# JackShDr/InfluentialRS

Measured on NVIDIA B200. Metric: IRN influence-path generation throughput @1M items, higher is better.
Workload: dtype f32

## Files before the change

influentialrs_b200/csrc/decoder_chain_tc.cu:

```cuda
#include "tc_common.cuh"
#include "qkv_image.cuh"

namespace irs {
namespace tcl {

using namespace irs::tc;

constexpr int BM = 128, D = 128, F = 256;
constexpr int RING = 4;
constexpr uint32_t UNIT_BYTES = 16384, UNIT_HALF = 8192;
constexpr uint32_t A_LBO = BM * 16;
constexpr uint32_t SBO = 128;
constexpr uint32_t OFF_P = 0;
constexpr uint32_t OFF_Q = 65536;
constexpr uint32_t OFF_RING = 131072;
constexpr uint32_t OFF_VEC = OFF_RING + RING * UNIT_BYTES;
constexpr int V_BO = 0, V_G1 = 128, V_B1 = 256, V_C2 = 384, V_G2 = 512, V_B2 = 640, V_BF1 = 768, V_BF2 = 1024,
              V_G3 = 1152, V_B3 = 1280, V_BIN = 1408, V_TOTAL = 1792;
constexpr uint32_t OFF_XCH = OFF_VEC + V_TOTAL * 4;
constexpr uint32_t OFF_BARS = OFF_XCH + 3 * 2 * 128 * 8;
enum Bars { B_FULL = 0, B_EMPTY = 4, B_A0 = 8, B_D1 = 9, B_A1 = 10, B_D2 = 11, B_A2 = 12 , B_D3 = 16,
            B_A3 = 17, B_D4 = 18, B_COUNT = 20 };
constexpr uint32_t OFF_TMEM = OFF_BARS + B_COUNT * 8;
constexpr uint32_t SMEM_BYTES = OFF_TMEM + 16;
constexpr int EPI_WARPS = 8, EPI_THREADS = EPI_WARPS * 32;
constexpr int LOAD_WARPS = 2;
constexpr int WARP_LOAD0 = 8, WARP_PROD = 10, WARP_MMA = 11;
constexpr int THREADS = 12 * 32;
constexpr int UNITS_BODY = 20;
constexpr int UNITS_QKV = 12;
constexpr uint32_t T_H = 0, T_Y = 256, T_D3 = 384;

struct Params {
  const float* attn;
  const float* x;
  float* x_out;
  float* qkv_out;
  uint8_t* qkv_images;
  int L, mask_mode;
  int qkv_only;
  const uint4* wstream;
  const float* vec[11];
  float eps1, eps2, eps3;
  int64_t R; int64_t n_tiles; int n_units;
  int* error_flag;
  long long* timeline;
};

struct UnitDesc { int mat, n0, k0, kind; };
__host__ __device__ inline UnitDesc unit_desc(int u) {
  UnitDesc d;
  if (u < 4) { d.mat = 0; d.n0 = 0; d.k0 = 32 * u; d.kind = 0; }
  else if (u < 12) { d.mat = 1; d.n0 = 0; d.k0 = 16 * (u - 4); d.kind = 2; }
  else if (u < 20) { d.mat = 2; d.n0 = 0; d.k0 = 32 * (u - 12); d.kind = 0; }
  else if (u < 28) { d.mat = 3; d.n0 = 0; d.k0 = 16 * (u - 20); d.kind = 2; }
  else { d.mat = 3; d.n0 = 256; d.k0 = 32 * (u - 28); d.kind = 0; }
  return d;
}

__global__ void __launch_bounds__(256)
prepare_chain_kernel(const float* __restrict__ Wo, const float* __restrict__ W1, const float* __restrict__ W2,
                     const float* __restrict__ Win, int n_units, uint4* __restrict__ out) {
  const int total = n_units * 1024;
  for (int idx = blockIdx.x * blockDim.x + threadIdx.x; idx < total; idx += gridDim.x * blockDim.x) {
    const int u = idx >> 10, w = idx & 1023;
    const int part = w >> 9, rem = w & 511;
    const UnitDesc ud = unit_desc(u);
    int slab, row;
    if (ud.kind == 0) { slab = rem >> 7; row = rem & 127; } else { slab = rem >> 8; row = rem & 255; }
    const float* W; int ldw;
    switch (ud.mat) { case 0: W = Wo; ldw = D; break; case 1: W = W1; ldw = D; break; case 2: W = W2; ldw = F; break;
                      default: W = Win; ldw = D; break; }
    const float* src = W + (int64_t)(ud.n0 + row) * ldw + ud.k0 + slab * 8;
    float x[8];
#pragma unroll
    for (int e = 0; e < 8; ++e) x[e] = src[e];
    uint4 hi, lo;
    split8(x, hi, lo);
    out[idx] = part ? lo : hi;
  }
}

__device__ __forceinline__ void ldg256_nc(const float* p, float (&a)[8]) {
  asm volatile("ld.global.nc.L1::no_allocate.v8.f32 {%0,%1,%2,%3,%4,%5,%6,%7}, [%8];"
               : "=f"(a[0]), "=f"(a[1]), "=f"(a[2]), "=f"(a[3]), "=f"(a[4]), "=f"(a[5]), "=f"(a[6]), "=f"(a[7]) : "l"(p));
}
__device__ __forceinline__ void ldg256(const float* p, float (&a)[8]) {
  asm volatile("ld.global.L1::no_allocate.v8.f32 {%0,%1,%2,%3,%4,%5,%6,%7}, [%8];"
               : "=f"(a[0]), "=f"(a[1]), "=f"(a[2]), "=f"(a[3]), "=f"(a[4]), "=f"(a[5]), "=f"(a[6]), "=f"(a[7]) : "l"(p) : "memory");
}
__device__ __forceinline__ void stg256(float* p, const float* a) {
  asm volatile("st.global.L1::no_allocate.v8.f32 [%0], {%1,%2,%3,%4,%5,%6,%7,%8};"
               :: "l"(p), "f"(a[0]), "f"(a[1]), "f"(a[2]), "f"(a[3]), "f"(a[4]), "f"(a[5]), "f"(a[6]), "f"(a[7]) : "memory");
}
__device__ __forceinline__ void stg128(void* p, const uint4& v) {
  asm volatile("st.global.L1::no_allocate.v4.b32 [%0], {%1,%2,%3,%4};" :: "l"(p), "r"(v.x), "r"(v.y), "r"(v.z), "r"(v.w) : "memory");
}
__device__ __forceinline__ void prefetch_l2_bulk(const void* p, uint32_t bytes) {
  asm volatile("cp.async.bulk.prefetch.L2.global [%0], %1;" :: "l"(p), "r"(bytes) : "memory");
}

template <int KSTEPS>
__device__ __forceinline__ void mma_unit(uint32_t d_tmem, uint32_t a_hi, uint32_t a_lo, uint32_t b_stage, uint32_t b_lbo,
                                         uint32_t idesc, bool first) {
#pragma unroll
  for (int kk = 0; kk < KSTEPS; ++kk) {
    const uint64_t ah = make_desc(a_hi + (uint32_t)(2 * kk) * A_LBO, A_LBO, SBO);
    const uint64_t al = make_desc(a_lo + (uint32_t)(2 * kk) * A_LBO, A_LBO, SBO);
    const uint64_t bh = make_desc(b_stage + (uint32_t)(2 * kk) * b_lbo, b_lbo, SBO);
    const uint64_t bl = make_desc(b_stage + UNIT_HALF + (uint32_t)(2 * kk) * b_lbo, b_lbo, SBO);
    tc_mma_bf16(d_tmem, al, bh, idesc, (first && kk == 0) ? 0u : 1u);
    tc_mma_bf16(d_tmem, ah, bl, idesc, 1u);
    tc_mma_bf16(d_tmem, ah, bh, idesc, 1u);
  }
}

#define IRS_TL(role, idx)                                                                         \
  do {                                                                                            \
    if (p.timeline && blockIdx.x == 0 && it < 8 && lane == 0)                                     \
      p.timeline[(it * 3 + (role)) * 32 + (idx)] = clock64();                                     \
  } while (0)

__device__ __forceinline__ void pair_barrier(int quad) {
  asm volatile("bar.sync %0, 64;" :: "r"(1 + quad) : "memory");
}

__device__ __forceinline__ float2 ln_pair_stats(float (&t)[64], float2* mine, const float2* other, int quad, float eps) {
  float s[4] = {0.f, 0.f, 0.f, 0.f}, q[4] = {0.f, 0.f, 0.f, 0.f};
#pragma unroll
  for (int j = 0; j < 64; ++j) s[j & 3] += t[j];
  const float m = ((s[0] + s[1]) + (s[2] + s[3])) * (1.0f / 64.0f);
#pragma unroll
  for (int j = 0; j < 64; ++j) {
    t[j] -= m;
    q[j & 3] = fmaf(t[j], t[j], q[j & 3]);
  }
  const float qs = (q[0] + q[1]) + (q[2] + q[3]);
  *mine = make_float2(m, qs);
  pair_barrier(quad);
  const float2 o = *other;
  const float delta = o.x - m;
  const float mean = 0.5f * (m + o.x);
  const float rstd = rsqrtf(fmaf(32.f * delta, delta, qs + o.y) * (1.0f / (float)D) + eps);
  return make_float2(rstd, (m - mean) * rstd);
}

__global__ void __launch_bounds__(THREADS, 1)
decoder_chain_kernel(const Params p) {
  extern __shared__ __align__(128) uint8_t smem[];
  const uint32_t sbase = smem_u32(smem);
  const int tid = threadIdx.x, warp = tid >> 5, lane = tid & 31;
  auto bar = [&](int i) { return sbase + OFF_BARS + 8u * (uint32_t)i; };
  volatile uint32_t* tmem_holder = reinterpret_cast<volatile uint32_t*>(smem + OFF_TMEM);
  float* vecs = reinterpret_cast<float*>(smem + OFF_VEC);
  const bool with_qkv = (p.qkv_out != nullptr) || (p.qkv_images != nullptr);
  const bool qkv_only = p.qkv_only != 0;

  if (tid == 0) {
    for (int s = 0; s < RING; ++s) { mbar_init(bar(B_FULL + s), 1); mbar_init(bar(B_EMPTY + s), 1); }
    mbar_init(bar(B_A0), LOAD_WARPS);
    mbar_init(bar(B_D1), 1);
    mbar_init(bar(B_A1), EPI_THREADS);
    mbar_init(bar(B_D2), 1);
    for (int i = 0; i < 4; ++i) mbar_init(bar(B_A2 + i), EPI_THREADS);
    mbar_init(bar(B_D3), 1);
    mbar_init(bar(B_A3), EPI_THREADS);
    for (int i = 0; i < 2; ++i) mbar_init(bar(B_D4 + i), 1);
    asm volatile("fence.mbarrier_init.release.cluster;" ::: "memory");
  }
  if (warp == WARP_MMA) {
    asm volatile("tcgen05.alloc.cta_group::1.sync.aligned.shared::cta.b32 [%0], %1;" :: "r"(sbase + OFF_TMEM), "r"(512u) : "memory");
    asm volatile("tcgen05.relinquish_alloc_permit.cta_group::1.sync.aligned;" ::: "memory");
  }
  {
    const int vlen[11] = {128, 128, 128, 128, 128, 128, 256, 128, 128, 128, 384};
    int off = 0;
    const float qscale0 = 1.4426950408889634f / sqrtf((float)img::DH);
    for (int v = 0; v < 11; ++v) {
      for (int i = tid; i < vlen[v]; i += THREADS) {
        float x = p.vec[v] ? p.vec[v][i] : 0.f;
        if (v == 2 && p.vec[3]) x += p.vec[3][i];
        if (v == 10 && p.qkv_images && i < D) x *= qscale0;
        vecs[off + i] = x;
      }
      off += vlen[v];
    }
  }
  tc_fence_before();
  __syncthreads();
  tc_fence_after();
  const uint32_t tmem_base = *tmem_holder;
  const int64_t first_tile = blockIdx.x, tile_step = gridDim.x;

  if (warp >= WARP_LOAD0 && warp < WARP_LOAD0 + LOAD_WARPS) {
    const int lw = warp - WARP_LOAD0;
    const int r8 = lane & 7, sg = lane >> 3;
    const uint32_t a0_off = qkv_only ? OFF_P : OFF_Q;
    int it = 0;
    for (int64_t tile = first_tile; tile < p.n_tiles; tile += tile_step, ++it) {
      const int64_t r0 = tile * BM;
#pragma unroll 1
      for (int batch = 0; batch < 64 / LOAD_WARPS / 8; ++batch) {
        float v[8][8];
#pragma unroll
        for (int q = 0; q < 8; ++q) {
          const int qq = batch * 8 + q;
          const int row = (lw * (16 / LOAD_WARPS) + (qq >> 2)) * 8 + r8;
          const int slab = (qq & 3) * 4 + sg;
          if (r0 + row < p.R) ldg256_nc(p.attn + (r0 + row) * D + slab * 8, v[q]);
          else {
#pragma unroll
            for (int e = 0; e < 8; ++e) v[q][e] = 0.f;
          }
        }
        if (batch == 0 && lw == 0) IRS_TL(2, 0);
        if (batch == 0 && it > 0) mbar_wait(bar(qkv_only ? B_D4 + 1 : B_D3), (uint32_t)((it - 1) & 1), p.error_flag, 31);
        if (batch == 0 && lw == 0) IRS_TL(2, 1);
#pragma unroll
        for (int q = 0; q < 8; ++q) {
          const int qq = batch * 8 + q;
          const int row = (lw * (16 / LOAD_WARPS) + (qq >> 2)) * 8 + r8;
          const int slab = (qq & 3) * 4 + sg;
          uint4 hi, lo;
          split8(v[q], hi, lo);
          *reinterpret_cast<uint4*>(smem + a0_off + slab * A_LBO + row * 16) = hi;
          *reinterpret_cast<uint4*>(smem + a0_off + 32768 + slab * A_LBO + row * 16) = lo;
        }
      }
      asm volatile("fence.proxy.async.shared::cta;" ::: "memory");
      __syncwarp();
      if (lane == 0) mbar_arrive(bar(B_A0));
      if (lw == 0) IRS_TL(2, 2);
    }
  } else if (warp == WARP_PROD) {
    if (lane == 0) {
      int64_t g = 0;
      for (int64_t tile = first_tile; tile < p.n_tiles; tile += tile_step) {
        const int64_t nt = tile + tile_step;
        if (nt < p.n_tiles) {
          const int64_t rows = (p.R - nt * BM) < BM ? (p.R - nt * BM) : BM;
          if (p.x) prefetch_l2_bulk(p.x + nt * BM * D, (uint32_t)(rows * D * 4));
          prefetch_l2_bulk(p.attn + nt * BM * D, (uint32_t)(rows * D * 4));
        }
        for (int u = 0; u < p.n_units; ++u, ++g) {
          const int stage = (int)(g % RING);
          const uint32_t phase = (uint32_t)((g / RING) & 1);
          mbar_wait(bar(B_EMPTY + stage), phase ^ 1u, p.error_flag, 32);
          mbar_arrive_expect_tx(bar(B_FULL + stage), UNIT_BYTES);
          bulk_g2s(sbase + OFF_RING + stage * UNIT_BYTES, p.wstream + (int64_t)u * (UNIT_BYTES / 16), UNIT_BYTES, bar(B_FULL + stage));
        }
      }
    }
  } else if (warp == WARP_MMA) {
    if (lane == 0) {
      const uint32_t idesc128 = make_idesc_bf16(BM, 128), idesc256 = make_idesc_bf16(BM, 256);
      const uint32_t P_HI = sbase + OFF_P, P_LO = sbase + OFF_P + 32768, Q_HI = sbase + OFF_Q, Q_LO = sbase + OFF_Q + 32768;
      int64_t g = 0;
      auto next_unit = [&]() -> uint32_t {
        const int stage = (int)(g % RING);
        mbar_wait(bar(B_FULL + stage), (uint32_t)((g / RING) & 1), p.error_flag, 33);
        tc_fence_after();
        return sbase + OFF_RING + stage * UNIT_BYTES;
      };
      auto release_unit = [&]() { tc_commit(bar(B_EMPTY + (int)(g % RING))); ++g; };
      int it = 0;
      for (int64_t tile = first_tile; tile < p.n_tiles; tile += tile_step, ++it) {
        const uint32_t ph = (uint32_t)(it & 1);
        if (qkv_only) {
          mbar_wait(bar(B_A0), ph, p.error_flag, 34);
          if (it > 0) mbar_wait(bar(B_A1), (uint32_t)((it - 1) & 1), p.error_flag, 38);
          tc_fence_after();
          for (int u = 0; u < 8; ++u) {
            const uint32_t bs = next_unit();
            mma_unit<1>(tmem_base + T_H, P_HI + (uint32_t)(2 * u) * A_LBO, P_LO + (uint32_t)(2 * u) * A_LBO, bs, 4096u, idesc256, u == 0);
            release_unit();
          }
          tc_commit(bar(B_D4 + 0));
          for (int c = 0; c < 4; ++c) {
            const uint32_t bs = next_unit();
            mma_unit<2>(tmem_base + T_D3, P_HI + (uint32_t)(4 * c) * A_LBO, P_LO + (uint32_t)(4 * c) * A_LBO, bs, 2048u, idesc128, c == 0);
            release_unit();
          }
          tc_commit(bar(B_D4 + 1));
          continue;
        }
        IRS_TL(0, 0);
        mbar_wait(bar(B_A0), ph, p.error_flag, 34);
        tc_fence_after();
        IRS_TL(0, 1);
        for (int c = 0; c < 4; ++c) {
          const uint32_t bs = next_unit();
          mma_unit<2>(tmem_base + T_Y, Q_HI + (uint32_t)(4 * c) * A_LBO, Q_LO + (uint32_t)(4 * c) * A_LBO, bs, 2048u, idesc128, c == 0);
          release_unit();
        }
        tc_commit(bar(B_D1));
        IRS_TL(0, 2);
        mbar_wait(bar(B_A1), ph, p.error_flag, 35);
        tc_fence_after();
        IRS_TL(0, 3);
        for (int u = 0; u < 8; ++u) {
          const uint32_t bs = next_unit();
          mma_unit<1>(tmem_base + T_H, P_HI + (uint32_t)(2 * u) * A_LBO, P_LO + (uint32_t)(2 * u) * A_LBO, bs, 4096u, idesc256, u == 0);
          release_unit();
        }
        tc_commit(bar(B_D2));
        for (int j = 0; j < 4; ++j) {
          IRS_TL(0, 4 + 2 * j);
          mbar_wait(bar(B_A2 + j), ph, p.error_flag, 36);
          tc_fence_after();
          IRS_TL(0, 5 + 2 * j);
          const uint32_t slot = (j < 2 ? Q_HI : P_HI) + (uint32_t)(j & 1) * 32768u;
          for (int i = 0; i < 2; ++i) {
            const uint32_t bs = next_unit();
            mma_unit<2>(tmem_base + T_D3, slot + (uint32_t)(4 * i) * A_LBO, slot + 16384u + (uint32_t)(4 * i) * A_LBO, bs,
                        2048u, idesc128, j == 0 && i == 0);
            release_unit();
          }
        }
        tc_commit(bar(B_D3));
        IRS_TL(0, 12);
        mbar_wait(bar(B_A3), ph, p.error_flag, 37);
        tc_fence_after();
        IRS_TL(0, 13);
        if (with_qkv) {
          for (int u = 0; u < 8; ++u) {
            const uint32_t bs = next_unit();
            mma_unit<1>(tmem_base + T_H, P_HI + (uint32_t)(2 * u) * A_LBO, P_LO + (uint32_t)(2 * u) * A_LBO, bs, 4096u, idesc256, u == 0);
            release_unit();
          }
          tc_commit(bar(B_D4 + 0));
          IRS_TL(0, 14);
          for (int c = 0; c < 4; ++c) {
            const uint32_t bs = next_unit();
            mma_unit<2>(tmem_base + T_D3, P_HI + (uint32_t)(4 * c) * A_LBO, P_LO + (uint32_t)(4 * c) * A_LBO, bs, 2048u, idesc128, c == 0);
            release_unit();
          }
          tc_commit(bar(B_D4 + 1));
          IRS_TL(0, 15);
        }
      }
    }
  } else if (warp < EPI_WARPS) {
    const int quad = warp & 3, half = warp >> 2;
    const int row = quad * 32 + lane;
    const uint32_t tlane = tmem_base + (((uint32_t)(quad * 32)) << 16);
    float2* xch = reinterpret_cast<float2*>(smem + OFF_XCH);
    const int c0 = half * 64;
    auto e4_piece = [&](int64_t tile, int it, int piece) {
      const uint32_t ph = (uint32_t)(it & 1);
      const int64_t r = tile * BM + row;
      const bool row_ok = r < p.R;
      float* qo = p.qkv_out ? p.qkv_out + (row_ok ? r : 0) * (3 * D) : nullptr;
      const int bb = (int)(r / p.L), ll = (int)(r - (int64_t)bb * p.L);
      const int n_chunks = (p.L + 31) / 32;
      const int qs = img::q_slot(n_chunks, ll);
      const uint32_t q_off = img::OFF_Q + (uint32_t)(qs / BM) * img::Q_TILE + (uint32_t)(qs % BM) * 16u;
      const uint32_t kv_off = (uint32_t)img::kv_col(p.mask_mode == IRS_MASK_PIM, p.L, ll) * 16u;
      uint8_t* item0 = p.qkv_images ? p.qkv_images + (int64_t)bb * (D / img::DH) * img::ITEM_BYTES : nullptr;
      const float qscale = 1.4426950408889634f / sqrtf((float)img::DH);
      {
      mbar_wait(bar(B_D4 + piece), ph, p.error_flag, 45);
      tc_fence_after();
      if (warp == 0) IRS_TL(1, 13 + 2 * piece);
      const int ncol = piece == 0 ? 128 : 64;
      const int col0 = piece == 0 ? half * 128 : 256 + half * 64;
      const uint32_t tcol = piece == 0 ? (T_H + (uint32_t)half * 128u) : (T_D3 + (uint32_t)half * 64u);
      auto emit = [&](const uint32_t (&v)[32], int ch) {
        float o32[32];
        const float sc = (p.qkv_images && col0 + ch * 32 < D) ? qscale : 1.0f;
#pragma unroll
        for (int j = 0; j < 32; ++j) o32[j] = fmaf(__uint_as_float(v[j]), sc, vecs[V_BIN + col0 + ch * 32 + j]);
        if (qo) {
          if (row_ok) {
#pragma unroll
            for (int q = 0; q < 4; ++q) stg256(qo + col0 + ch * 32 + q * 8, &o32[q * 8]);
          }
        } else if (row_ok) {
          const int c = col0 + ch * 32;
          const int which = c >> 7, head = (c & 127) >> 5;
          uint8_t* dst = item0 + (int64_t)head * img::ITEM_BYTES + (which == 0 ? q_off : (which == 1 ? img::OFF_K : img::OFF_V) + kv_off);
          const uint32_t lbo = which == 0 ? img::Q_LBO : img::K_LBO, part = which == 0 ? img::Q_PART : img::K_PART;
#pragma unroll
          for (int s8 = 0; s8 < 4; ++s8) {
            uint4 hi, lo;
            split8(*reinterpret_cast<float(*)[8]>(&o32[s8 * 8]), hi, lo);
            stg128(dst + s8 * lbo, hi);
            stg128(dst + part + s8 * lbo, lo);
          }
        }
      };
      {
        const int nch = ncol / 32;
        uint32_t va[32], vb[32];
        tc_ld32(tlane + tcol, va);
#pragma unroll 1
        for (int ch = 0; ch < nch; ch += 2) {
          tc_wait_ld();
          if (ch + 1 < nch) tc_ld32(tlane + tcol + (ch + 1) * 32, vb);
          emit(va, ch);
          if (ch + 1 < nch) {
            tc_wait_ld();
            if (ch + 2 < nch) tc_ld32(tlane + tcol + (ch + 2) * 32, va);
            emit(vb, ch + 1);
          }
        }
      }
      if (warp == 0) IRS_TL(1, 14 + 2 * piece);
      }
    };
    int it = 0;
    for (int64_t tile = first_tile; tile < p.n_tiles; tile += tile_step, ++it) {
      const uint32_t ph = (uint32_t)(it & 1);
      const int64_t r = tile * BM + row;
      const bool row_ok = r < p.R;
      if (!qkv_only) {
      float t[64];
      {
        const float* xrow = p.x + (row_ok ? r : 0) * D + c0;
#pragma unroll
        for (int q = 0; q < 8; ++q) {
          if (row_ok) ldg256(xrow + q * 8, *reinterpret_cast<float(*)[8]>(&t[q * 8]));
          else {
#pragma unroll
            for (int e = 0; e < 8; ++e) t[q * 8 + e] = 0.f;
          }
        }
      }
      if (warp == 0) IRS_TL(1, 0);
      mbar_wait(bar(B_D1), ph, p.error_flag, 41);
      tc_fence_after();
      if (warp == 0) IRS_TL(1, 1);
#pragma unroll
      for (int ch = 0; ch < 2; ++ch) {
        uint32_t v[32];
        tc_ld32(tlane + T_Y + c0 + ch * 32, v);
        tc_wait_ld();
#pragma unroll
        for (int j = 0; j < 32; ++j) {
          t[ch * 32 + j] = __uint_as_float(v[j]) + vecs[V_BO + c0 + ch * 32 + j] + t[ch * 32 + j];
        }
      }
      const float2 st1 = ln_pair_stats(t, &xch[(0 * 2 + half) * 128 + row], &xch[(0 * 2 + (half ^ 1)) * 128 + row],
                                       quad, p.eps1);
#pragma unroll
      for (int j = 0; j < 64; ++j) {
        const int n = c0 + j;
        t[j] = fmaf(fmaf(t[j], st1.x, st1.y), vecs[V_G1 + n], vecs[V_B1 + n]);
      }
      const float2 st2 = ln_pair_stats(t, &xch[(1 * 2 + half) * 128 + row], &xch[(1 * 2 + (half ^ 1)) * 128 + row],
                                       quad, p.eps2);
#pragma unroll
      for (int ch = 0; ch < 2; ++ch) {
        uint32_t v[32];
#pragma unroll
        for (int j = 0; j < 32; ++j) {
          const int n = c0 + ch * 32 + j;
          const float y = fmaf(fmaf(t[ch * 32 + j], st2.x, st2.y), vecs[V_G2 + n], vecs[V_B2 + n]);
          t[ch * 32 + j] = y;
          v[j] = __float_as_uint(y);
        }
        tc_st32(tlane + T_Y + c0 + ch * 32, v);
#pragma unroll
        for (int s8 = 0; s8 < 4; ++s8) {
          uint4 hi, lo;
          split8(*reinterpret_cast<float(*)[8]>(&t[ch * 32 + s8 * 8]), hi, lo);
          const uint32_t o = (uint32_t)(half * 8 + ch * 4 + s8) * A_LBO + (uint32_t)row * 16u;
          *reinterpret_cast<uint4*>(smem + OFF_P + o) = hi;
          *reinterpret_cast<uint4*>(smem + OFF_P + 32768 + o) = lo;
        }
      }
      tc_wait_st();
      asm volatile("fence.proxy.async.shared::cta;" ::: "memory");
      tc_fence_before();
      mbar_arrive(bar(B_A1));
      if (warp == 0) IRS_TL(1, 2);
      if (with_qkv && it > 0) e4_piece(tile - tile_step, it - 1, 1);
      mbar_wait(bar(B_D2), ph, p.error_flag, 42);
      tc_fence_after();
#pragma unroll 1
      for (int j = 0; j < 4; ++j) {
        uint32_t v[32];
        tc_ld32(tlane + T_H + 64u * (uint32_t)j + 32u * (uint32_t)half, v);
        if (warp == 0) IRS_TL(1, 3 + 2 * j);
        uint8_t* slot = smem + (j < 2 ? OFF_Q : OFF_P) + (j & 1) * 32768;
        tc_wait_ld();
#pragma unroll
        for (int s8 = 0; s8 < 4; ++s8) {
          float x8[8];
#pragma unroll
          for (int e = 0; e < 8; ++e)
            x8[e] = fmaxf(__uint_as_float(v[s8 * 8 + e]) + vecs[V_BF1 + j * 64 + half * 32 + s8 * 8 + e], 0.f);
          uint4 hi, lo;
          split8(x8, hi, lo);
          const uint32_t o = (uint32_t)(half * 4 + s8) * A_LBO + (uint32_t)row * 16u;
          *reinterpret_cast<uint4*>(slot + o) = hi;
          *reinterpret_cast<uint4*>(slot + 16384 + o) = lo;
        }
        asm volatile("fence.proxy.async.shared::cta;" ::: "memory");
        tc_fence_before();
        mbar_arrive(bar(B_A2 + j));
        if (warp == 0) IRS_TL(1, 4 + 2 * j);
      }
      mbar_wait(bar(B_D3), ph, p.error_flag, 44);
      tc_fence_after();
      if (warp == 0) IRS_TL(1, 11);
#pragma unroll
      for (int ch = 0; ch < 2; ++ch) {
        uint32_t v[32], y[32];
        tc_ld32(tlane + T_D3 + c0 + ch * 32, v);
        tc_ld32(tlane + T_Y + c0 + ch * 32, y);
        tc_wait_ld();
#pragma unroll
        for (int j = 0; j < 32; ++j) {
          t[ch * 32 + j] = __uint_as_float(v[j]) + vecs[V_BF2 + c0 + ch * 32 + j] + __uint_as_float(y[j]);
        }
      }
      const float2 st3 = ln_pair_stats(t, &xch[(2 * 2 + half) * 128 + row], &xch[(2 * 2 + (half ^ 1)) * 128 + row],
                                       quad, p.eps3);
      float* xo = p.x_out + (row_ok ? r : 0) * D + c0;
#pragma unroll
      for (int ch = 0; ch < 2; ++ch) {
#pragma unroll
        for (int j = 0; j < 32; ++j) {
          const int n = c0 + ch * 32 + j;
          t[ch * 32 + j] = fmaf(fmaf(t[ch * 32 + j], st3.x, st3.y), vecs[V_G3 + n], vecs[V_B3 + n]);
        }
        if (row_ok) {
#pragma unroll
          for (int q = 0; q < 4; ++q) stg256(xo + ch * 32 + q * 8, &t[ch * 32 + q * 8]);
        }
        if (with_qkv) {
#pragma unroll
          for (int s8 = 0; s8 < 4; ++s8) {
            uint4 hi, lo;
            split8(*reinterpret_cast<float(*)[8]>(&t[ch * 32 + s8 * 8]), hi, lo);
            const uint32_t o = (uint32_t)(half * 8 + ch * 4 + s8) * A_LBO + (uint32_t)row * 16u;
            *reinterpret_cast<uint4*>(smem + OFF_P + o) = hi;
            *reinterpret_cast<uint4*>(smem + OFF_P + 32768 + o) = lo;
          }
        }
      }
      if (with_qkv) asm volatile("fence.proxy.async.shared::cta;" ::: "memory");
      tc_fence_before();
      mbar_arrive(bar(B_A3));
      if (warp == 0) IRS_TL(1, 12);
      }
      if (qkv_only) {
        e4_piece(tile, it, 0);
        e4_piece(tile, it, 1);
        tc_fence_before();
        mbar_arrive(bar(B_A1));
      } else if (with_qkv) {
        e4_piece(tile, it, 0);
      }
      tc_fence_before();
    }
    if (!qkv_only && with_qkv && it > 0) e4_piece(first_tile + (int64_t)(it - 1) * tile_step, it - 1, 1);
    tc_fence_before();
  }

  tc_fence_before();
  __syncthreads();
  if (warp == WARP_MMA) {
    tc_fence_after();
    asm volatile("tcgen05.dealloc.cta_group::1.sync.aligned.b32 %0, %1;" :: "r"(tmem_base), "r"(512u) : "memory");
  }
}

}
}

using namespace irs;

static long long* g_chain_timeline = nullptr;

extern "C" void irs_decoder_chain_debug_timeline(long long* buf) { g_chain_timeline = buf; }

extern "C" int irs_decoder_chain_supported(int d, int ffn) { return (d == tcl::D && ffn == tcl::F) ? 1 : 0; }

extern "C" size_t irs_decoder_chain_prepared_bytes(int d, int ffn, int with_in_proj) {
  if (!irs_decoder_chain_supported(d, ffn)) return 0;
  return (size_t)(tcl::UNITS_BODY + (with_in_proj ? tcl::UNITS_QKV : 0)) * tcl::UNIT_BYTES;
}

extern "C" int irs_decoder_chain_prepare_weights(const float* Wo, const float* W1, const float* W2, const float* Win,
                                                 int d, int ffn, void* prepared, void* stream) {
  if (!Wo || !W1 || !W2 || !prepared) return IRS_E_BADARG;
  if (!irs_decoder_chain_supported(d, ffn)) return IRS_E_SHAPE;
  const int n_units = tcl::UNITS_BODY + (Win ? tcl::UNITS_QKV : 0);
  tcl::prepare_chain_kernel<<<64, 256, 0, (cudaStream_t)stream>>>(Wo, W1, W2, Win, n_units, (uint4*)prepared);
  IRS_LAUNCHED();
  return 0;
}

static int chain_launch(tcl::Params& p, int64_t R, int* error_flag, void* stream) {
  p.R = R; p.n_tiles = ceil_div(R, tcl::BM);
  p.error_flag = error_flag;
  p.timeline = g_chain_timeline;
  static bool configured = false;
  if (!configured) {
    IRS_CUDA(cudaFuncSetAttribute(tcl::decoder_chain_kernel, cudaFuncAttributeMaxDynamicSharedMemorySize, (int)tcl::SMEM_BYTES));
    configured = true;
  }
  const unsigned grid = (unsigned)(p.n_tiles < kNumSMs ? p.n_tiles : kNumSMs);
  tcl::decoder_chain_kernel<<<grid, tcl::THREADS, tcl::SMEM_BYTES, (cudaStream_t)stream>>>(p);
  IRS_LAUNCHED();
  return 0;
}

extern "C" int irs_decoder_chain_tc(const float* attn, const float* x, const void* prepared,
                                    const float* bo, const float* g1, const float* b1, const float* c2,
                                    const float* g2, const float* b2, const float* bf1, const float* bf2,
                                    const float* g3, const float* b3, const float* bin,
                                    float eps1, float eps2, float eps3,
                                    float* x_out, float* qkv_out, void* qkv_images, int L, int mask_mode,
                                    int64_t R, int d, int ffn, int* error_flag, void* stream) {
  if (!attn || !x || !prepared || !x_out || !g1 || !b1 || !g2 || !b2 || !g3 || !b3) return IRS_E_BADARG;
  if (R < 0 || (qkv_out && qkv_images)) return IRS_E_BADARG;
  if (R == 0) return 0;
  if (!irs_decoder_chain_supported(d, ffn)) return IRS_E_SHAPE;
  if (qkv_images && (L <= 128 || L > irs::img::KEYS - 1 || R % L != 0 || mask_mode < 0 || mask_mode > 2)) return IRS_E_SHAPE;
  if (((uintptr_t)attn & 31) || ((uintptr_t)x & 31) || ((uintptr_t)x_out & 31) || ((uintptr_t)qkv_out & 31) ||
      ((uintptr_t)qkv_images & 15) || ((uintptr_t)prepared & 15))
    return IRS_E_SHAPE;
  tcl::Params p = {};
  p.attn = attn; p.x = x; p.x_out = x_out; p.qkv_out = qkv_out; p.qkv_images = (uint8_t*)qkv_images;
  p.L = qkv_images ? L : 1; p.mask_mode = mask_mode; p.qkv_only = 0;
  p.wstream = (const uint4*)prepared;
  const float* vec[11] = {bo, g1, b1, c2, g2, b2, bf1, bf2, g3, b3, bin};
  for (int i = 0; i < 11; ++i) p.vec[i] = vec[i];
  p.eps1 = eps1; p.eps2 = eps2; p.eps3 = eps3;
  p.n_units = tcl::UNITS_BODY + ((qkv_out || qkv_images) ? tcl::UNITS_QKV : 0);
  return chain_launch(p, R, error_flag, stream);
}

extern "C" int irs_in_proj_images_tc(const float* x, const void* prepared_with_in_proj, const float* bin,
                                     void* qkv_images, int L, int mask_mode, int64_t R, int d,
                                     int* error_flag, void* stream) {
  if (!x || !prepared_with_in_proj || !qkv_images) return IRS_E_BADARG;
  if (R < 0) return IRS_E_BADARG;
  if (R == 0) return 0;
  if (d != tcl::D) return IRS_E_SHAPE;
  if (L <= 128 || L > irs::img::KEYS - 1 || R % L != 0 || mask_mode < 0 || mask_mode > 2) return IRS_E_SHAPE;
  if (((uintptr_t)x & 31) || ((uintptr_t)qkv_images & 15) || ((uintptr_t)prepared_with_in_proj & 15)) return IRS_E_SHAPE;
  tcl::Params p = {};
  p.attn = x; p.x = nullptr; p.x_out = nullptr; p.qkv_out = nullptr; p.qkv_images = (uint8_t*)qkv_images;
  p.L = L; p.mask_mode = mask_mode; p.qkv_only = 1;
  p.wstream = (const uint4*)prepared_with_in_proj + (size_t)tcl::UNITS_BODY * (tcl::UNIT_BYTES / 16);
  p.vec[10] = bin;
  p.n_units = tcl::UNITS_QKV;
  return chain_launch(p, R, error_flag, stream);
}
```

Baseline: 388,500.

## Split epilogue-to-MMA handoffs into per-chunk barriers to overlap tensor-core work

Result: no change. 388,000 (median of 6 runs) (-0.1%).

```diff
diff --git a/influentialrs_b200/csrc/decoder_chain_tc.cu b/influentialrs_b200/csrc/decoder_chain_tc.cu
--- a/influentialrs_b200/csrc/decoder_chain_tc.cu
+++ b/influentialrs_b200/csrc/decoder_chain_tc.cu
@@ -1,5 +1,6 @@
 #include "tc_common.cuh"
 #include "qkv_image.cuh"
+
 
 namespace irs {
 namespace tcl {
@@ -19,8 +20,8 @@
               V_G3 = 1152, V_B3 = 1280, V_BIN = 1408, V_TOTAL = 1792;
 constexpr uint32_t OFF_XCH = OFF_VEC + V_TOTAL * 4;
 constexpr uint32_t OFF_BARS = OFF_XCH + 3 * 2 * 128 * 8;
-enum Bars { B_FULL = 0, B_EMPTY = 4, B_A0 = 8, B_D1 = 9, B_A1 = 10, B_D2 = 11, B_A2 = 12 , B_D3 = 16,
-            B_A3 = 17, B_D4 = 18, B_COUNT = 20 };
+enum Bars { B_FULL = 0, B_EMPTY = 4, B_A0 = 8, B_D1 = 9, B_A1 = 10, B_D2 = 14, B_A2 = 15 ,
+            B_D3 = 19, B_A3 = 20, B_D4 = 24, B_QF = 27, B_COUNT = 28 };
 constexpr uint32_t OFF_TMEM = OFF_BARS + B_COUNT * 8;
 constexpr uint32_t SMEM_BYTES = OFF_TMEM + 16;
 constexpr int EPI_WARPS = 8, EPI_THREADS = EPI_WARPS * 32;
@@ -53,8 +54,7 @@
   if (u < 4) { d.mat = 0; d.n0 = 0; d.k0 = 32 * u; d.kind = 0; }
   else if (u < 12) { d.mat = 1; d.n0 = 0; d.k0 = 16 * (u - 4); d.kind = 2; }
   else if (u < 20) { d.mat = 2; d.n0 = 0; d.k0 = 32 * (u - 12); d.kind = 0; }
-  else if (u < 28) { d.mat = 3; d.n0 = 0; d.k0 = 16 * (u - 20); d.kind = 2; }
-  else { d.mat = 3; d.n0 = 256; d.k0 = 32 * (u - 28); d.kind = 0; }
+  else { d.mat = 3; d.n0 = 128 * ((u - 20) >> 2); d.k0 = 32 * ((u - 20) & 3); d.kind = 0; }
   return d;
 }
 
@@ -115,11 +115,12 @@
   }
 }
 
-#define IRS_TL(role, idx)                                                                         \
+#define IRS_TL_AT(tile_it, role, idx)                                                             \
   do {                                                                                            \
-    if (p.timeline && blockIdx.x == 0 && it < 8 && lane == 0)                                     \
-      p.timeline[(it * 3 + (role)) * 32 + (idx)] = clock64();                                     \
+    if (p.timeline && blockIdx.x == 0 && (tile_it) < 8 && lane == 0)                              \
+      p.timeline[((tile_it) * 3 + (role)) * 32 + (idx)] = clock64();                              \
   } while (0)
+#define IRS_TL(role, idx) IRS_TL_AT(it, role, idx)
 
 __device__ __forceinline__ void pair_barrier(int quad) {
   asm volatile("bar.sync %0, 64;" :: "r"(1 + quad) : "memory");
@@ -160,12 +161,13 @@
     for (int s = 0; s < RING; ++s) { mbar_init(bar(B_FULL + s), 1); mbar_init(bar(B_EMPTY + s), 1); }
     mbar_init(bar(B_A0), LOAD_WARPS);
     mbar_init(bar(B_D1), 1);
-    mbar_init(bar(B_A1), EPI_THREADS);
+    for (int i = 0; i < 4; ++i) mbar_init(bar(B_A1 + i), EPI_THREADS / 2);
     mbar_init(bar(B_D2), 1);
     for (int i = 0; i < 4; ++i) mbar_init(bar(B_A2 + i), EPI_THREADS);
     mbar_init(bar(B_D3), 1);
-    mbar_init(bar(B_A3), EPI_THREADS);
-    for (int i = 0; i < 2; ++i) mbar_init(bar(B_D4 + i), 1);
+    for (int i = 0; i < 4; ++i) mbar_init(bar(B_A3 + i), EPI_THREADS / 2);
+    for (int i = 0; i < 3; ++i) mbar_init(bar(B_D4 + i), 1);
+    mbar_init(bar(B_QF), 1);
     asm volatile("fence.mbarrier_init.release.cluster;" ::: "memory");
   }
   if (warp == WARP_MMA) {
@@ -195,13 +197,11 @@
   if (warp >= WARP_LOAD0 && warp < WARP_LOAD0 + LOAD_WARPS) {
     const int lw = warp - WARP_LOAD0;
     const int r8 = lane & 7, sg = lane >> 3;
-    const uint32_t a0_off = qkv_only ? OFF_P : OFF_Q;
     int it = 0;
     for (int64_t tile = first_tile; tile < p.n_tiles; tile += tile_step, ++it) {
       const int64_t r0 = tile * BM;
-#pragma unroll 1
-      for (int batch = 0; batch < 64 / LOAD_WARPS / 8; ++batch) {
-        float v[8][8];
+      const uint32_t a0_off = qkv_only ? OFF_P : OFF_Q;
+      auto load = [&](int batch, float (&v)[8][8]) {
 #pragma unroll
         for (int q = 0; q < 8; ++q) {
           const int qq = batch * 8 + q;
@@ -213,9 +213,8 @@
             for (int e = 0; e < 8; ++e) v[q][e] = 0.f;
           }
         }
-        if (batch == 0 && lw == 0) IRS_TL(2, 0);
-        if (batch == 0 && it > 0) mbar_wait(bar(qkv_only ? B_D4 + 1 : B_D3), (uint32_t)((it - 1) & 1), p.error_flag, 31);
-        if (batch == 0 && lw == 0) IRS_TL(2, 1);
+      };
+      auto store = [&](int batch, const float (&v)[8][8]) {
 #pragma unroll
         for (int q = 0; q < 8; ++q) {
           const int qq = batch * 8 + q;
@@ -226,6 +225,20 @@
           *reinterpret_cast<uint4*>(smem + a0_off + slab * A_LBO + row * 16) = hi;
           *reinterpret_cast<uint4*>(smem + a0_off + 32768 + slab * A_LBO + row * 16) = lo;
         }
+      };
+      constexpr int BATCHES = 64 / LOAD_WARPS / 8;
+      float v[2][8][8];
+      load(0, v[0]);
+      if (lw == 0) IRS_TL(2, 0);
+      if (it > 0) {
+        mbar_wait(bar(qkv_only ? B_D4 + 2 : B_QF), (uint32_t)((it - 1) & 1), p.error_flag, 31);
+      }
+      if (lw == 0) IRS_TL(2, 1);
+      store(0, v[0]);
+#pragma unroll 1
+      for (int batch = 1; batch < BATCHES; ++batch) {
+        load(batch, v[0]);
+        store(batch, v[0]);
       }
       asm volatile("fence.proxy.async.shared::cta;" ::: "memory");
       __syncwarp();
@@ -263,25 +276,47 @@
         return sbase + OFF_RING + stage * UNIT_BYTES;
       };
       auto release_unit = [&]() { tc_commit(bar(B_EMPTY + (int)(g % RING))); ++g; };
+      int ready = 0;
+      auto need_group = [&](int b, int grp, uint32_t ph, int code, int it, int tl0) {
+        for (; ready <= grp; ++ready) {
+          mbar_wait(bar(b + ready), ph, p.error_flag, code);
+          tc_fence_after();
+          IRS_TL_AT(it, 0, tl0 + ready);
+        }
+      };
+      auto in_proj_qk = [&](bool groups, uint32_t ph, int it, uint32_t A_HI, uint32_t A_LO) {
+        ready = 0;
+        for (int h = 0; h < 2; ++h) {
+          for (int c = 0; c < 4; ++c) {
+            if (groups) need_group(B_A3, c, ph, 37, it, 18);
+            const uint32_t bs = next_unit();
+            mma_unit<2>(tmem_base + T_H + 128u * (uint32_t)h, A_HI + (uint32_t)(4 * c) * A_LBO, A_LO + (uint32_t)(4 * c) * A_LBO,
+                        bs, 2048u, idesc128, c == 0);
+            release_unit();
+          }
+          tc_commit(bar(B_D4 + h));
+          IRS_TL_AT(it, 0, 22 + h);
+        }
+      };
+      auto in_proj_v = [&](int it, uint32_t A_HI, uint32_t A_LO) {
+        for (int c = 0; c < 4; ++c) {
+          const uint32_t bs = next_unit();
+          mma_unit<2>(tmem_base + T_D3, A_HI + (uint32_t)(4 * c) * A_LBO, A_LO + (uint32_t)(4 * c) * A_LBO, bs, 2048u, idesc128, c == 0);
+          release_unit();
+        }
+        tc_commit(bar(B_D4 + 2));
+        IRS_TL_AT(it, 0, 24);
+      };
       int it = 0;
       for (int64_t tile = first_tile; tile < p.n_tiles; tile += tile_step, ++it) {
         const uint32_t ph = (uint32_t)(it & 1);
         if (qkv_only) {
           mbar_wait(bar(B_A0), ph, p.error_flag, 34);
-          if (it > 0) mbar_wait(bar(B_A1), (uint32_t)((it - 1) & 1), p.error_flag, 38);
+          if (it > 0)
+            for (int i = 0; i < 4; ++i) mbar_wait(bar(B_A1 + i), (uint32_t)((it - 1) & 1), p.error_flag, 38);
           tc_fence_after();
-          for (int u = 0; u < 8; ++u) {
-            const uint32_t bs = next_unit();
-            mma_unit<1>(tmem_base + T_H, P_HI + (uint32_t)(2 * u) * A_LBO, P_LO + (uint32_t)(2 * u) * A_LBO, bs, 4096u, idesc256, u == 0);
-            release_unit();
-          }
-          tc_commit(bar(B_D4 + 0));
-          for (int c = 0; c < 4; ++c) {
-            const uint32_t bs = next_unit();
-            mma_unit<2>(tmem_base + T_D3, P_HI + (uint32_t)(4 * c) * A_LBO, P_LO + (uint32_t)(4 * c) * A_LBO, bs, 2048u, idesc128, c == 0);
-            release_unit();
-          }
-          tc_commit(bar(B_D4 + 1));
+          in_proj_qk(false, ph, it, P_HI, P_LO);
+          in_proj_v(it, P_HI, P_LO);
           continue;
         }
         IRS_TL(0, 0);
@@ -295,20 +330,20 @@
         }
         tc_commit(bar(B_D1));
         IRS_TL(0, 2);
-        mbar_wait(bar(B_A1), ph, p.error_flag, 35);
-        tc_fence_after();
-        IRS_TL(0, 3);
+        ready = 0;
         for (int u = 0; u < 8; ++u) {
+          need_group(B_A1, u >> 1, ph, 35, it, 3);
           const uint32_t bs = next_unit();
           mma_unit<1>(tmem_base + T_H, P_HI + (uint32_t)(2 * u) * A_LBO, P_LO + (uint32_t)(2 * u) * A_LBO, bs, 4096u, idesc256, u == 0);
           release_unit();
         }
         tc_commit(bar(B_D2));
+        IRS_TL(0, 8);
         for (int j = 0; j < 4; ++j) {
-          IRS_TL(0, 4 + 2 * j);
+          IRS_TL(0, 9 + 2 * j);
           mbar_wait(bar(B_A2 + j), ph, p.error_flag, 36);
           tc_fence_after();
-          IRS_TL(0, 5 + 2 * j);
+          IRS_TL(0, 10 + 2 * j);
           const uint32_t slot = (j < 2 ? Q_HI : P_HI) + (uint32_t)(j & 1) * 32768u;
           for (int i = 0; i < 2; ++i) {
             const uint32_t bs = next_unit();
@@ -316,27 +351,16 @@
                         2048u, idesc128, j == 0 && i == 0);
             release_unit();
           }
+          if (j == 1) tc_commit(bar(B_QF));
         }
         tc_commit(bar(B_D3));
-        IRS_TL(0, 12);
-        mbar_wait(bar(B_A3), ph, p.error_flag, 37);
-        tc_fence_after();
-        IRS_TL(0, 13);
+        IRS_TL(0, 17);
         if (with_qkv) {
-          for (int u = 0; u < 8; ++u) {
-            const uint32_t bs = next_unit();
-            mma_unit<1>(tmem_base + T_H, P_HI + (uint32_t)(2 * u) * A_LBO, P_LO + (uint32_t)(2 * u) * A_LBO, bs, 4096u, idesc256, u == 0);
-            release_unit();
-          }
-          tc_commit(bar(B_D4 + 0));
-          IRS_TL(0, 14);
-          for (int c = 0; c < 4; ++c) {
-            const uint32_t bs = next_unit();
-            mma_unit<2>(tmem_base + T_D3, P_HI + (uint32_t)(4 * c) * A_LBO, P_LO + (uint32_t)(4 * c) * A_LBO, bs, 2048u, idesc128, c == 0);
-            release_unit();
-          }
-          tc_commit(bar(B_D4 + 1));
-          IRS_TL(0, 15);
+          in_proj_qk(true, ph, it, P_HI, P_LO);
+          in_proj_v(it, P_HI, P_LO);
+        } else {
+          ready = 0;
+          need_group(B_A3, 3, ph, 37, it, 18);
         }
       }
     }
@@ -359,9 +383,11 @@
       uint8_t* item0 = p.qkv_images ? p.qkv_images + (int64_t)bb * (D / img::DH) * img::ITEM_BYTES : nullptr;
       const float qscale = 1.4426950408889634f / sqrtf((float)img::DH);
       {
-      mbar_wait(bar(B_D4 + piece), ph, p.error_flag, 45);
+      const int tl = piece == 0 ? 16 + 2 * half : 20;
+      mbar_wait(bar(piece == 0 ? B_D4 + half : B_D4 + 2), ph, p.error_flag, 45);
       tc_fence_after();
-      if (warp == 0) IRS_TL(1, 13 + 2 * piece);
+      const bool tl_warp = (warp & 3) == 0 && (piece == 0 || half == 0);
+      if (tl_warp) IRS_TL(1, tl);
       const int ncol = piece == 0 ? 128 : 64;
       const int col0 = piece == 0 ? half * 128 : 256 + half * 64;
       const uint32_t tcol = piece == 0 ? (T_H + (uint32_t)half * 128u) : (T_D3 + (uint32_t)half * 64u);
@@ -405,7 +431,7 @@
           }
         }
       }
-      if (warp == 0) IRS_TL(1, 14 + 2 * piece);
+      if (tl_warp) IRS_TL(1, tl + 1);
       }
     };
     int it = 0;
@@ -451,15 +477,11 @@
                                        quad, p.eps2);
 #pragma unroll
       for (int ch = 0; ch < 2; ++ch) {
-        uint32_t v[32];
 #pragma unroll
         for (int j = 0; j < 32; ++j) {
           const int n = c0 + ch * 32 + j;
-          const float y = fmaf(fmaf(t[ch * 32 + j], st2.x, st2.y), vecs[V_G2 + n], vecs[V_B2 + n]);
-          t[ch * 32 + j] = y;
-          v[j] = __float_as_uint(y);
-        }
-        tc_st32(tlane + T_Y + c0 + ch * 32, v);
+          t[ch * 32 + j] = fmaf(fmaf(t[ch * 32 + j], st2.x, st2.y), vecs[V_G2 + n], vecs[V_B2 + n]);
+        }
 #pragma unroll
         for (int s8 = 0; s8 < 4; ++s8) {
           uint4 hi, lo;
@@ -468,12 +490,20 @@
           *reinterpret_cast<uint4*>(smem + OFF_P + o) = hi;
           *reinterpret_cast<uint4*>(smem + OFF_P + 32768 + o) = lo;
         }
+        asm volatile("fence.proxy.async.shared::cta;" ::: "memory");
+        tc_fence_before();
+        mbar_arrive(bar(B_A1 + 2 * half + ch));
+        if (warp == 0 && ch == 0) IRS_TL(1, 2);
+      }
+#pragma unroll
+      for (int ch = 0; ch < 2; ++ch) {
+        uint32_t v[32];
+#pragma unroll
+        for (int j = 0; j < 32; ++j) v[j] = __float_as_uint(t[ch * 32 + j]);
+        tc_st32(tlane + T_Y + c0 + ch * 32, v);
       }
       tc_wait_st();
-      asm volatile("fence.proxy.async.shared::cta;" ::: "memory");
-      tc_fence_before();
-      mbar_arrive(bar(B_A1));
-      if (warp == 0) IRS_TL(1, 2);
+      if (warp == 0) IRS_TL(1, 3);
       if (with_qkv && it > 0) e4_piece(tile - tile_step, it - 1, 1);
       mbar_wait(bar(B_D2), ph, p.error_flag, 42);
       tc_fence_after();
@@ -481,7 +511,7 @@
       for (int j = 0; j < 4; ++j) {
         uint32_t v[32];
         tc_ld32(tlane + T_H + 64u * (uint32_t)j + 32u * (uint32_t)half, v);
-        if (warp == 0) IRS_TL(1, 3 + 2 * j);
+        if (warp == 0) IRS_TL(1, 4 + 2 * j);
         uint8_t* slot = smem + (j < 2 ? OFF_Q : OFF_P) + (j & 1) * 32768;
         tc_wait_ld();
 #pragma unroll
@@ -499,11 +529,11 @@
         asm volatile("fence.proxy.async.shared::cta;" ::: "memory");
         tc_fence_before();
         mbar_arrive(bar(B_A2 + j));
-        if (warp == 0) IRS_TL(1, 4 + 2 * j);
+        if (warp == 0) IRS_TL(1, 5 + 2 * j);
       }
       mbar_wait(bar(B_D3), ph, p.error_flag, 44);
       tc_fence_after();
-      if (warp == 0) IRS_TL(1, 11);
+      if (warp == 0) IRS_TL(1, 12);
 #pragma unroll
       for (int ch = 0; ch < 2; ++ch) {
         uint32_t v[32], y[32];
@@ -517,17 +547,12 @@
       }
       const float2 st3 = ln_pair_stats(t, &xch[(2 * 2 + half) * 128 + row], &xch[(2 * 2 + (half ^ 1)) * 128 + row],
                                        quad, p.eps3);
-      float* xo = p.x_out + (row_ok ? r : 0) * D + c0;
 #pragma unroll
       for (int ch = 0; ch < 2; ++ch) {
 #pragma unroll
         for (int j = 0; j < 32; ++j) {
           const int n = c0 + ch * 32 + j;
           t[ch * 32 + j] = fmaf(fmaf(t[ch * 32 + j], st3.x, st3.y), vecs[V_G3 + n], vecs[V_B3 + n]);
-        }
-        if (row_ok) {
-#pragma unroll
-          for (int q = 0; q < 4; ++q) stg256(xo + ch * 32 + q * 8, &t[ch * 32 + q * 8]);
         }
         if (with_qkv) {
 #pragma unroll
@@ -538,18 +563,26 @@
             *reinterpret_cast<uint4*>(smem + OFF_P + o) = hi;
             *reinterpret_cast<uint4*>(smem + OFF_P + 32768 + o) = lo;
           }
-        }
-      }
-      if (with_qkv) asm volatile("fence.proxy.async.shared::cta;" ::: "memory");
-      tc_fence_before();
-      mbar_arrive(bar(B_A3));
-      if (warp == 0) IRS_TL(1, 12);
+          asm volatile("fence.proxy.async.shared::cta;" ::: "memory");
+        }
+        tc_fence_before();
+        mbar_arrive(bar(B_A3 + 2 * half + ch));
+        if (warp == 0 && ch == 0) IRS_TL(1, 13);
+      }
+      if (warp == 0) IRS_TL(1, 14);
+      if (row_ok) {
+        float* xo = p.x_out + r * D + c0;
+#pragma unroll
+        for (int q = 0; q < 8; ++q) stg256(xo + q * 8, &t[q * 8]);
+      }
+      if (warp == 0) IRS_TL(1, 15);
       }
       if (qkv_only) {
         e4_piece(tile, it, 0);
         e4_piece(tile, it, 1);
         tc_fence_before();
-        mbar_arrive(bar(B_A1));
+        mbar_arrive(bar(B_A1 + 2 * half));
+        mbar_arrive(bar(B_A1 + 2 * half + 1));
       } else if (with_qkv) {
         e4_piece(tile, it, 0);
       }
```
